# RRr89/Shared_SIMD_Scan

Measured on AMD Instinct MI355X. Metric: scanned values/sec + achieved HBM GB/s, 1e9 x 9-bit column (equality scan, bitmap + hit count out), higher is better.
Workload: dtype u32; 1 GPU; scan_eq ONE 1e+09x9bit column in 1 row-range shard(s) of <= 1000000000 rows, column=mod5, key=3; rows_total=1000000000, bits=9, parallelism=row-range shards x1

## Files before the change

shared_simd_scan_amd/csrc/kernels/in_list.hpp:

```cpp
#pragma once

#include "scan.hpp"

namespace mi355 {

template <int C, int AUX_, int VPL>
__global__ __launch_bounds__(kBlockThreads) void in_kernel(ScanArgs a)
{
    using G = ScanGeom<C, VPL>;
    constexpr int WORDS = G::WORDS;
    constexpr int AUX = AUX_ & 15;
    constexpr int NTS = store_policy_of(AUX_);
    constexpr bool BITSET = C <= 16;
    constexpr int SET_BYTES = BITSET ? ((1 << (C < 16 ? C : 16)) + 7) / 8 : 16;
    __shared__ __attribute__((aligned(16))) uint8_t lds[kWavesPerBlock][G::LDS_BYTES];
    __shared__ __attribute__((aligned(16))) uint32_t set_words[(SET_BYTES + 3) / 4];
    __shared__ __attribute__((aligned(16))) uint8_t mlds[kWavesPerBlock][1024];

    const int lane = threadIdx.x & 63;
    const int wave = __builtin_amdgcn_readfirstlane(threadIdx.x >> 6);
    uint8_t *lds_wave = lds[wave];
    const TileCtx<C, VPL> tc(a.n);
    const uint64_t stride = (uint64_t)gridDim.x * kWavesPerBlock;
    uint64_t tile = (uint64_t)blockIdx.x * kWavesPerBlock + wave;
// ... 19 lines not shown
    }
    const uint8_t *set_bytes = (const uint8_t *)set_words;

    uint32_t hits = 0;
    uint32_t res[WORDS];
    uint64_t prev = ~0ull;
    uint8_t *const out_lane = a.out + lane * (WORDS * 4);
    while (tile < tc.ntiles) {
        asm volatile("s_waitcnt vmcnt(0)" ::: "memory");
        uint32_t w[G::LANE_DWORDS];
        read_lane_data<C, VPL>(lds_wave, lane, w);
        uint32_t mcur[WORDS];
        if (a.and_mask && tile < tc.nfull) {
#pragma unroll
            for (int j = 0; j < WORDS; j++) mcur[j] = ((const uint32_t *)(mlds_wave + lane * (WORDS * 4)))[j];
        }
        asm volatile("s_waitcnt lgkmcnt(0)" ::: "memory");
        if (prev != ~0ull) store_words<WORDS, NTS>(out_lane + prev * G::BITMAP_BYTES, res);
        const uint64_t next = tile + stride;
        if (next < tc.ntiles) issue_tile(next);

        uint32_t xs[VPL];
        extract_all<C, VPL, 0, G::LANE_DWORDS>(w, xs);
        if constexpr (BITSET) {
#pragma unroll
            for (int j = 0; j < WORDS; j++) {
                uint32_t acc = 0;
#pragma unroll
                for (int k = 31; k >= 0; k--) {
                    const uint32_t x = xs[32 * j + k];
                    const uint32_t bit = (set_bytes[x >> 3] >> (x & 7)) & 1u;
                    acc = (acc << 1) | bit;
                }
                res[j] = acc;
            }
        } else {
            uint32_t m[WORDS];
#pragma unroll
            for (int j = 0; j < WORDS; j++) m[j] = 0;
            for (uint32_t k = 0; k < P; k++) {
                const uint32_t key = __builtin_amdgcn_readfirstlane((uint32_t)a.keys_dev[k]);
#pragma unroll
                for (int j = 0; j < WORDS; j++) {
                    uint32_t acc = 0;
#pragma unroll
                    for (int i = 31; i >= 0; i--) acc = (acc << 1) | (xs[32 * j + i] == key ? 1u : 0u);
                    m[j] |= acc;
                }
            }
#pragma unroll
            for (int j = 0; j < WORDS; j++) res[j] = m[j];
        }
        const uint32_t inv = a.invert;
#pragma unroll
        for (int j = 0; j < WORDS; j++) res[j] ^= inv;
        if (tile < tc.nfull) {
            if (a.and_mask) {
#pragma unroll
                for (int j = 0; j < WORDS; j++) res[j] &= mcur[j];
            }
#pragma unroll
            for (int j = 0; j < WORDS; j++) hits += __builtin_popcount(res[j]);
            prev = tile;
        } else {
            const int64_t left = (int64_t)(tc.n - tile * G::TILE_VALUES) - (int64_t)lane * VPL;
            const int nbytes = left <= 0 ? 0 : (int)((left >= VPL ? VPL : left) + 7) / 8;
            if (a.and_mask) {
                const uint8_t *mp = a.and_mask + tile * G::BITMAP_BYTES + lane * (WORDS * 4);
#pragma unroll
                for (int j = 0; j < WORDS; j++) {
                    uint32_t mm = 0;
#pragma unroll
                    for (int b = 0; b < 4; b++)
                        if (4 * j + b < nbytes) mm |= (uint32_t)mp[4 * j + b] << (8 * b);
                    res[j] &= mm;
                }
            }
            hits += tc.finish_tail(tile, res, out_lane + tile * G::BITMAP_BYTES, 1, lane);
            prev = ~0ull;
        }
        tile = next;
    }
    if (prev != ~0ull) store_words<WORDS, NTS>(out_lane + prev * G::BITMAP_BYTES, res);
    if (a.hits) hits_add(a, 0, wave_sum(hits), lane);
    hits_finalize(a, 1, lane);
}

}
```

shared_simd_scan_amd/csrc/kernels/scan.hpp:

```cpp
#pragma once

#include "tile.hpp"

namespace mi355 {

template <int C, int VPL> struct TileCtx {
    using G = ScanGeom<C, VPL>;
    uint64_t n, ntiles, nfull, data_bytes;
    uint32_t llc_inv, llc_lim;
    __device__ __forceinline__ TileCtx(uint64_t n_, uint32_t llc_inv_ = 0, uint32_t llc_lim_ = 0) : n(n_), llc_inv(llc_inv_), llc_lim(llc_lim_)
    {
        ntiles = (n + G::TILE_VALUES - 1) / G::TILE_VALUES;
        nfull = n / G::TILE_VALUES;
        data_bytes = (n * C + 7) / 8;
    }
    template <int AUX> __device__ __forceinline__ void issue(const uint8_t *packed, uint64_t t, uint8_t *lds_wave, int lane) const
    {
        if constexpr (AUX != 0) {
            if (llc_inv != 0 && (uint32_t)((t * G::TILE_BYTES) >> kLlcGranuleShift) * llc_inv <= llc_lim) {
                issue_as<0>(packed, t, lds_wave, lane);
                return;
            }
        }
        issue_as<AUX>(packed, t, lds_wave, lane);
    }
    template <int AUX> __device__ __forceinline__ void issue_as(const uint8_t *packed, uint64_t t, uint8_t *lds_wave, int lane) const
    {
        const uint8_t *src = packed + t * G::TILE_BYTES;
        if (t < nfull)
            dma_tile_full<G::TILE_BYTES, AUX>(src, lds_wave, lane);
        else
            dma_tile_partial<G::TILE_BYTES, AUX>(src, data_bytes - t * G::TILE_BYTES, lds_wave, lane);
    }
    template <bool HAVE_NBYTES = false>
    __device__ __forceinline__ void load_bitmap_words(const uint8_t *bits, uint64_t t, int lane, uint32_t (&m)[VPL / 32], uint64_t have_nbytes = 0) const
    {
        constexpr int WORDS = G::WORDS;
        const uint64_t at = t * G::BITMAP_BYTES + (uint64_t)lane * (WORDS * 4);
        if (t < nfull) {
#pragma unroll
            for (int j = 0; j < WORDS; j++) m[j] = ((const uint32_t *)(bits + at))[j];
        } else {
            const uint64_t nbytes = HAVE_NBYTES ? have_nbytes : (n + 7) / 8;
#pragma unroll
            for (int j = 0; j < WORDS; j++) {
                uint32_t v = 0;
#pragma unroll
                for (int b = 0; b < 4; b++)
                    if (at + 4 * j + b < nbytes) v |= (uint32_t)bits[at + 4 * j + b] << (8 * b);
                m[j] = v;
            }
        }
    }
    __device__ __forceinline__ uint32_t finish_tail(uint64_t t, uint32_t (&v)[VPL / 32], uint8_t *dst, uint64_t byte_stride, int lane,
                                                    bool store = true) const
    {
        const int64_t left = (int64_t)(n - t * G::TILE_VALUES) - (int64_t)lane * VPL;
        const int valid = left >= VPL ? VPL : (left <= 0 ? 0 : (int)left);
        const int nbytes = (valid + 7) / 8;
        uint32_t cnt = 0;
#pragma unroll
        for (int j = 0; j < VPL / 32; j++) {
            v[j] &= tail_mask(valid, j);
            cnt += __builtin_popcount(v[j]);
#pragma unroll
            for (int b = 0; b < 4; b++)
                if (store && 4 * j + b < nbytes) dst[(uint64_t)(4 * j + b) * byte_stride] = (uint8_t)(v[j] >> (8 * b));
        }
        return cnt;
    }
};

template <int C, int VPL, int K> constexpr int burst_occ()
{
    using G = ScanGeom<C, VPL>;
    constexpr int mask_bytes = (K * G::BITMAP_BYTES + 1023) / 1024 * 1024;
    constexpr int table = narrow_k<C>() ? (1 << (narrow_k<C>() * C)) : 16;
    constexpr int lds = kCuLdsBytes / (4 * (G::LDS_BYTES + mask_bytes) + table + 64);
    constexpr int cap = narrow_k<C>() ? 4 : 8;
    return lds > cap ? cap : (lds < 1 ? 1 : lds);
}

template <int C, int MODE, int AUX_, int VPL, int K>
__global__ __launch_bounds__(kBlockThreads, (burst_occ<C, VPL, K>())) void scan_burst_kernel(ScanArgs a)
{
    using G = ScanGeom<C, VPL>;
    static_assert(MODE == kModeEq || MODE == kModeRange, "MODE");
    constexpr int WORDS = G::WORDS;
    constexpr int AUX = AUX_ & 15;
    constexpr int NTS = store_policy_of(AUX_);
    __shared__ __attribute__((aligned(16))) uint8_t lds[kWavesPerBlock][G::LDS_BYTES];
    constexpr int LK = narrow_k<C>();
    __shared__ __attribute__((aligned(16))) uint8_t nlut[LK ? (1 << (LK * C)) : 16];
    constexpr int MASK_DMA = (K * G::BITMAP_BYTES + 1023) / 1024;
    __shared__ __attribute__((aligned(16))) uint8_t mlds[kWavesPerBlock][MASK_DMA * 1024];

    const int lane = threadIdx.x & 63;
    const int wave = __builtin_amdgcn_readfirstlane(threadIdx.x >> 6);
    uint8_t *lds_wave = lds[wave];
    uint8_t *mlds_wave = mlds[wave];
    const TileCtx<C, VPL> tc(a.n, a.llc_inv, a.llc_lim);
    const uint64_t nchunks = (tc.ntiles + K - 1) / K;
    const uint64_t stride = (uint64_t)gridDim.x * kWavesPerBlock;
    uint64_t chunk = (uint64_t)blockIdx.x * kWavesPerBlock + wave;

    uint32_t key[2] = {a.key[0], a.key[1]};
    uint32_t hits = 0;
    uint8_t *const out_lane = a.out + lane * (WORDS * 4);
    const bool store = a.out != nullptr;
    const uint8_t *const mask = a.and_mask;
    const uint32_t mop = a.mask_op, inv = a.invert;
    auto combine = [mop](uint32_t r, uint32_t m) -> uint32_t {
        return mop == 0 ? (r & m) : mop == 1 ? (r | m) : mop == 2 ? (r ^ m) : (m & ~r);
    };

    uint32_t res[K][WORDS];
    uint64_t pend_chunk = 0;
    int pend_n = 0;

    if (chunk < nchunks) tc.template issue<AUX>(a.packed, chunk * K, lds_wave, lane);
    if constexpr (LK > 0) {
        constexpr uint32_t fmask = (1u << C) - 1u;
        for (uint32_t e = threadIdx.x; e < (1u << (LK * C)); e += kBlockThreads) {
            uint32_t m = 0;
#pragma unroll
            for (int j = 0; j < LK; j++) {
                const uint32_t f = (e >> (j * C)) & fmask;
                const bool hit = (MODE == kModeRange) ? (f - key[0]) <= key[1] : f == key[0];
                m |= (hit ? 1u : 0u) << j;
            }
            nlut[e] = (uint8_t)m;
        }
        __syncthreads();
    }

    while (chunk < nchunks) {
        const uint64_t tfirst = chunk * K;
        int nfull_here = 0;
#pragma unroll
        for (int k = 0; k < K; k++) {
            const uint64_t tile = tfirst + k;
            if (tile < tc.ntiles) {
                asm volatile("s_waitcnt vmcnt(0)" ::: "memory");
                uint32_t w[G::LANE_DWORDS];
                read_lane_data<C, VPL>(lds_wave, lane, w);
                uint32_t mcur[WORDS];
                if (k > 0 && mask) {
#pragma unroll
                    for (int j = 0; j < WORDS; j++) mcur[j] = ((const uint32_t *)(mlds_wave + k * G::BITMAP_BYTES + lane * (WORDS * 4)))[j];
                }
                asm volatile("s_waitcnt lgkmcnt(0)" ::: "memory");
                if (k == 0) {
                    if (pend_n && store) {
                        uint8_t *dst = out_lane + pend_chunk * K * G::BITMAP_BYTES;
#pragma unroll
                        for (int q = 0; q < K; q++)
                            if (q < pend_n) store_words<WORDS, NTS>(dst + q * G::BITMAP_BYTES, res[q]);
                    }
                    pend_n = 0;
                    if (mask) {
                        const uint64_t mbytes = (tc.nfull > tfirst ? (tc.nfull - tfirst < K ? tc.nfull - tfirst : K) : 0) * G::BITMAP_BYTES;
                        const uint8_t *src = mask + tfirst * G::BITMAP_BYTES;
#pragma unroll
                        for (int q = 0; q < MASK_DMA; q++) {
                            const uint32_t o = q * 1024 + lane * 16;
                            if (o < mbytes) __builtin_amdgcn_global_load_lds(MI355_GPTR(src + o), MI355_LPTR(mlds_wave + q * 1024), 16, 0, 0);
                        }
                    }
                }
                const uint64_t next = (k + 1 < K && tile + 1 < tc.ntiles) ? tile + 1 : (chunk + stride) * K;
                const bool have_next = next < tc.ntiles && (k + 1 < K || chunk + stride < nchunks);
                if (have_next) tc.template issue<AUX>(a.packed, next, lds_wave, lane);
                uint32_t r1[1][WORDS];
                if constexpr (LK > 0) {
                    decode_words_narrow<C, VPL, LK, 0, G::LANE_DWORDS>(w, r1, nlut);
                } else {
                    const uint32_t key8[kMaxKeysPerPass] = {key[0], key[1], 0, 0, 0, 0, 0, 0};
                    decode_words<C, VPL, 0, 1, MODE, G::LANE_DWORDS>(w, r1, key8);
                }
#pragma unroll
                for (int j = 0; j < WORDS; j++) r1[0][j] ^= inv;
                if (tile < tc.nfull) {
                    if (mask) {
                        if (k == 0) {
                            if (have_next && next < tc.nfull)
                                asm volatile("s_waitcnt vmcnt(%0)" ::"n"(G::DMA_INSTRS) : "memory");
                            else
                                asm volatile("s_waitcnt vmcnt(0)" ::: "memory");
#pragma unroll
                            for (int j = 0; j < WORDS; j++) mcur[j] = ((const uint32_t *)(mlds_wave + lane * (WORDS * 4)))[j];
                            asm volatile("s_waitcnt lgkmcnt(0)" ::: "memory");
                        }
#pragma unroll
                        for (int j = 0; j < WORDS; j++) r1[0][j] = combine(r1[0][j], mcur[j]);
                    }
#pragma unroll
                    for (int j = 0; j < WORDS; j++) {
                        hits += __builtin_popcount(r1[0][j]);
                        res[k][j] = r1[0][j];
                    }
                    nfull_here = k + 1;
                } else {
                    if (mask) {
                        const uint8_t *mp = mask + tile * G::BITMAP_BYTES + lane * (WORDS * 4);
                        const int64_t left = (int64_t)(tc.n - tile * G::TILE_VALUES) - (int64_t)lane * VPL;
                        const int nbytes = left <= 0 ? 0 : (int)((left >= VPL ? VPL : left) + 7) / 8;
#pragma unroll
                        for (int j = 0; j < WORDS; j++) {
                            uint32_t m = 0;
#pragma unroll
                            for (int b = 0; b < 4; b++)
                                if (4 * j + b < nbytes) m |= (uint32_t)mp[4 * j + b] << (8 * b);
                            r1[0][j] = combine(r1[0][j], m);
                        }
                    }
                    hits += tc.finish_tail(tile, r1[0], out_lane + tile * G::BITMAP_BYTES, 1, lane, store);
                }
            }
        }
        pend_chunk = chunk;
        pend_n = nfull_here;
        chunk += stride;
    }
    if (pend_n && store) {
        uint8_t *dst = out_lane + pend_chunk * K * G::BITMAP_BYTES;
#pragma unroll
        for (int q = 0; q < K; q++)
            if (q < pend_n) store_words<WORDS, NTS>(dst + q * G::BITMAP_BYTES, res[q]);
    }
    if (a.hits) hits_add(a, 0, wave_sum(hits), lane);
    hits_finalize(a, 1, lane);
}

template <int C, int AUX_, int VPL>
__global__ __launch_bounds__(kBlockThreads, (burst_occ<C, VPL, 1>() > 1 ? burst_occ<C, VPL, 1>() / 2 : 1)) void scan2_kernel(ScanArgs a)
{
    using G = ScanGeom<C, VPL>;
    constexpr int WORDS = G::WORDS;
    constexpr int AUX = AUX_ & 15;
    constexpr int NTS = store_policy_of(AUX_);
    __shared__ __attribute__((aligned(16))) uint8_t lds[kWavesPerBlock][2][G::LDS_BYTES];

    const int lane = threadIdx.x & 63;
    const int wave = __builtin_amdgcn_readfirstlane(threadIdx.x >> 6);
    uint8_t *lds1 = lds[wave][0], *lds2 = lds[wave][1];
    const TileCtx<C, VPL> tc(a.n);
    const uint64_t stride = (uint64_t)gridDim.x * kWavesPerBlock;
    uint64_t tile = (uint64_t)blockIdx.x * kWavesPerBlock + wave;
    const uint32_t k1[kMaxKeysPerPass] = {a.key[0], a.key[1], 0, 0, 0, 0, 0, 0};
    const uint32_t k2[kMaxKeysPerPass] = {a.key2[0], a.key2[1], 0, 0, 0, 0, 0, 0};
    const uint32_t inv1 = a.invert, inv2 = a.invert2, mop = a.mask_op;
    auto combine = [mop](uint32_t p2, uint32_t p1) -> uint32_t {
        return mop == 0 ? (p2 & p1) : mop == 1 ? (p2 | p1) : mop == 2 ? (p2 ^ p1) : (p1 & ~p2);
    };
    uint32_t hits = 0;
    uint8_t *const out_lane = a.out + lane * (WORDS * 4);
    const bool store = a.out != nullptr;
    uint32_t res[WORDS];
    uint64_t prev = ~0ull;

    auto issue = [&](uint64_t t) {
        tc.template issue<AUX>(a.packed, t, lds1, lane);
        tc.template issue<AUX>(a.packed2, t, lds2, lane);
    };
    if (tile < tc.ntiles) issue(tile);
    while (tile < tc.ntiles) {
        asm volatile("s_waitcnt vmcnt(0)" ::: "memory");
        uint32_t w1[G::LANE_DWORDS], w2[G::LANE_DWORDS];
        read_lane_data<C, VPL>(lds1, lane, w1);
        read_lane_data<C, VPL>(lds2, lane, w2);
        asm volatile("s_waitcnt lgkmcnt(0)" ::: "memory");
        if (prev != ~0ull && store) store_words<WORDS, NTS>(out_lane + prev * G::BITMAP_BYTES, res);
        const uint64_t next = tile + stride;
        if (next < tc.ntiles) issue(next);
        uint32_t r1[1][WORDS], r2[1][WORDS];
        decode_words<C, VPL, 0, 1, kModeRange, G::LANE_DWORDS>(w1, r1, k1);
        decode_words<C, VPL, 0, 1, kModeRange, G::LANE_DWORDS>(w2, r2, k2);
#pragma unroll
        for (int j = 0; j < WORDS; j++) res[j] = combine(r2[0][j] ^ inv2, r1[0][j] ^ inv1);
        if (tile < tc.nfull) {
#pragma unroll
            for (int j = 0; j < WORDS; j++) hits += __builtin_popcount(res[j]);
            prev = tile;
        } else {
            hits += tc.finish_tail(tile, res, out_lane + tile * G::BITMAP_BYTES, 1, lane, store);
            prev = ~0ull;
        }
        tile = next;
    }
    if (prev != ~0ull && store) store_words<WORDS, NTS>(out_lane + prev * G::BITMAP_BYTES, res);
    if (a.hits) hits_add(a, 0, wave_sum(hits), lane);
    hits_finalize(a, 1, lane);
}

__device__ __forceinline__ void transpose4x4_bytes(const uint32_t (&r)[4], uint32_t (&c)[4])
{
    const uint32_t t0 = __builtin_amdgcn_perm(r[1], r[0], 0x05010400u);
    const uint32_t t1 = __builtin_amdgcn_perm(r[1], r[0], 0x07030602u);
    const uint32_t t2 = __builtin_amdgcn_perm(r[3], r[2], 0x05010400u);
    const uint32_t t3 = __builtin_amdgcn_perm(r[3], r[2], 0x07030602u);
    c[0] = __builtin_amdgcn_perm(t2, t0, 0x05040100u);
    c[1] = __builtin_amdgcn_perm(t2, t0, 0x07060302u);
    c[2] = __builtin_amdgcn_perm(t3, t1, 0x05040100u);
    c[3] = __builtin_amdgcn_perm(t3, t1, 0x07060302u);
}

}
```

shared_simd_scan_amd/csrc/kernels/tile.hpp:

```cpp
#pragma once

#include <hip/hip_runtime.h>
#include <stdint.h>

#include "../switches.hpp"

namespace mi355 {

typedef uint32_t u32x4 __attribute__((ext_vector_type(4)));
typedef uint32_t u32x2 __attribute__((ext_vector_type(2)));

#define MI355_GPTR(p) ((const __attribute__((address_space(1))) void *)(p))
#define MI355_LPTR(p) ((__attribute__((address_space(3))) void *)(p))

constexpr int kWavesPerBlock = 4;
constexpr int kBlockThreads = kWavesPerBlock * 64;
constexpr int kCuLdsBytes = 160 * 1024;
constexpr int kMaxKeysPerPass = 8;
constexpr uint64_t value_reach(unsigned c, uint64_t count) { return (c < 32 && count > (1ull << c)) ? (1ull << c) : count; }
constexpr int kMaxKeys = 1024;

template <int C, int VPL> struct ScanGeom {
    static_assert(VPL == 32 || VPL == 64 || VPL == 128, "VPL");
    static constexpr int WORDS = VPL / 32;
// ... 334 lines not shown
{
    Unaligned64 v;
    v.lo = lo;
    v.hi = hi;
    *(Unaligned64 *)dst = v;
}

constexpr int store_policy_of(int aux) { return (aux & 32) ? 2 : ((aux & 16) ? 1 : 0); }

template <int WORDS, int NT = 0> __device__ __forceinline__ void store_words(uint8_t *dst, const uint32_t (&v)[WORDS])
{
    if constexpr (WORDS == 4) {
        u32x4 t = {v[0], v[1], v[2], v[3]};
        if constexpr (NT == 2) {
            asm volatile("global_store_dwordx4 %0, %1, off sc1" ::"v"(dst), "v"(t) : "memory");
        } else if constexpr (NT == 1) __builtin_nontemporal_store(t, (u32x4 *)dst); else *(u32x4 *)dst = t;
    } else if constexpr (WORDS == 2) {
        u32x2 t = {v[0], v[1]};
        if constexpr (NT == 2) {
            asm volatile("global_store_dwordx2 %0, %1, off sc1" ::"v"(dst), "v"(t) : "memory");
        } else if constexpr (NT == 1) __builtin_nontemporal_store(t, (u32x2 *)dst); else *(u32x2 *)dst = t;
    } else {
        if constexpr (NT) __builtin_nontemporal_store(v[0], (uint32_t *)dst); else *(uint32_t *)dst = v[0];
    }
}

constexpr int kHitSlots = 64;
constexpr int kDoneGroups = 16;
constexpr int kScratchWords = kHitSlots * kMaxKeys + 8 + kDoneGroups * 16;
constexpr int kScratchDone = kHitSlots * kMaxKeys;
constexpr int kScratchGroupDone = kScratchDone + 8;

__device__ __forceinline__ void hits_add(const ScanArgs &a, uint32_t k, uint32_t wave_total, int lane)
{
    if (lane == 0 && wave_total)
        __hip_atomic_fetch_add(a.scratch + (blockIdx.x % kHitSlots) * kMaxKeys + k, (unsigned long long)wave_total,
                               __ATOMIC_RELAXED, __HIP_MEMORY_SCOPE_AGENT);
}

__device__ __forceinline__ void hits_finalize(const ScanArgs &a, uint32_t P, int lane)
{
    if (!a.hits) return;
    __shared__ uint32_t s_last;
    asm volatile("s_waitcnt vmcnt(0)" ::: "memory");
    __syncthreads();
    if (threadIdx.x == 0) {
        const uint32_t g = blockIdx.x % kDoneGroups;
        const uint32_t in_group = (gridDim.x - g + kDoneGroups - 1) / kDoneGroups;
        const uint32_t ngroups = gridDim.x < (unsigned)kDoneGroups ? gridDim.x : (unsigned)kDoneGroups;
        unsigned long long *const gdone = a.scratch + kScratchGroupDone + g * 16;
        uint32_t last = 0;
        if (__hip_atomic_fetch_add(gdone, 1ull, __ATOMIC_RELAXED, __HIP_MEMORY_SCOPE_AGENT) == (unsigned long long)in_group - 1) {
            __hip_atomic_store(gdone, 0ull, __ATOMIC_RELAXED, __HIP_MEMORY_SCOPE_AGENT);
            last = __hip_atomic_fetch_add(a.scratch + kScratchDone, 1ull, __ATOMIC_RELAXED, __HIP_MEMORY_SCOPE_AGENT) == (unsigned long long)ngroups - 1;
        }
        s_last = last;
    }
    __syncthreads();
    if (s_last) {
        const uint32_t nslots = gridDim.x < (unsigned)kHitSlots ? gridDim.x : (unsigned)kHitSlots;
        if (P <= 16u) {
            for (uint32_t k = threadIdx.x >> 6; k < P; k += kBlockThreads / 64) {
                const unsigned long long v = (uint32_t)lane < nslots
                                                 ? __hip_atomic_exchange(a.scratch + (uint32_t)lane * kMaxKeys + k, 0ull, __ATOMIC_RELAXED, __HIP_MEMORY_SCOPE_AGENT)
                                                 : 0ull;
                const unsigned long long lo = wave_sum((uint32_t)(v & 0xffffffull)), mid = wave_sum((uint32_t)((v >> 24) & 0xffffffull)),
                                         hi = wave_sum((uint32_t)(v >> 48));
                if (lane == 0) a.hits[k] = lo + (mid << 24) + (hi << 48);
            }
            if (threadIdx.x == 0) __hip_atomic_store(a.scratch + kScratchDone, 0ull, __ATOMIC_RELAXED, __HIP_MEMORY_SCOPE_AGENT);
            return;
        }
        for (uint32_t k = threadIdx.x; k < P; k += kBlockThreads) {
            unsigned long long v = 0;
#pragma unroll 8
            for (uint32_t sl = 0; sl < nslots; sl++)
                v += __hip_atomic_exchange(a.scratch + sl * kMaxKeys + k, 0ull, __ATOMIC_RELAXED, __HIP_MEMORY_SCOPE_AGENT);
            a.hits[k] = v;
        }
        if (threadIdx.x == 0) __hip_atomic_store(a.scratch + kScratchDone, 0ull, __ATOMIC_RELAXED, __HIP_MEMORY_SCOPE_AGENT);
    }
}

__device__ __forceinline__ void block_hits_clear(uint32_t *s_hits)
{
    for (uint32_t k = threadIdx.x; k < (uint32_t)kMaxKeys; k += kBlockThreads) s_hits[k] = 0;
}
__device__ __forceinline__ void block_hits_add8(uint32_t *s_hits, uint32_t kbase, uint32_t P, const uint32_t (&cnt)[8], int lane)
{
    uint32_t p0 = cnt[0] | (cnt[1] << 16), p1 = cnt[2] | (cnt[3] << 16), p2 = cnt[4] | (cnt[5] << 16), p3 = cnt[6] | (cnt[7] << 16);
    p0 = wave_sum(p0);
    p1 = wave_sum(p1);
    p2 = wave_sum(p2);
    p3 = wave_sum(p3);
    if (lane == 0) {
        const uint32_t v[8] = {p0 & 0xffff, p0 >> 16, p1 & 0xffff, p1 >> 16, p2 & 0xffff, p2 >> 16, p3 & 0xffff, p3 >> 16};
#pragma unroll
        for (int q = 0; q < 8; q++)
            if (kbase + q < P && v[q]) atomicAdd(&s_hits[kbase + q], v[q]);
    }
}

__device__ __forceinline__ void block_hits_flush(const ScanArgs &a, uint32_t *s_hits, uint32_t P)
{
    __syncthreads();
    for (uint32_t k = threadIdx.x; k < P; k += blockDim.x) {
        const uint32_t v = s_hits[k];
        if (v)
            __hip_atomic_fetch_add(a.scratch + (blockIdx.x % kHitSlots) * kMaxKeys + k, (unsigned long long)v, __ATOMIC_RELAXED,
                                   __HIP_MEMORY_SCOPE_AGENT);
    }
}

template <int C, int LK, int J, int GI, int NW>
__device__ __forceinline__ void narrow_step(const uint32_t (&w)[NW], uint32_t &acc, const uint8_t *table)
{
    constexpr int FIRST = LK * GI;
    constexpr int LEN = (32 - FIRST) < LK ? (32 - FIRST) : LK;
    uint32_t m = table[extract_at<(32 * J + FIRST) * C, LEN * C, NW>(w)];
    if constexpr (LEN < LK) m &= (1u << LEN) - 1u;
    acc = (acc << LEN) | m;
    if constexpr (GI > 0) narrow_step<C, LK, J, GI - 1, NW>(w, acc, table);
}

template <int C, int VPL, int LK, int J, int NW>
__device__ __forceinline__ void decode_words_narrow(const uint32_t (&w)[NW], uint32_t (&res)[1][VPL / 32], const uint8_t *table)
{
    uint32_t acc = 0;
    narrow_step<C, LK, J, (32 + LK - 1) / LK - 1, NW>(w, acc, table);
    res[0][J] = acc;
    if constexpr (J + 1 < VPL / 32) decode_words_narrow<C, VPL, LK, J + 1, NW>(w, res, table);
}

}
```

shared_simd_scan_amd/csrc/predicates/columns.hpp:

```cpp
#pragma once

#include "../kernels.hpp"
#include "../kernels/rt_column.hpp"

namespace mi355 {

struct ColumnsArgs {
    ScanArgs s;
    uint32_t c2;
    uint32_t nts;
    uint32_t lo, span;
    int64_t lo64;
    uint64_t span64;
};

constexpr int kColumnsMaskLds = 1024;

constexpr int columns_vpl(int C, bool same) { return same ? scan_vpl(C, kModeRange) : 32; }
template <int C1, int VPL, bool SAME> constexpr uint32_t columns_wave_lds(uint32_t c2)
{
    return (uint32_t)ScanGeom<C1, VPL>::LDS_BYTES + (SAME ? 1u : 2u) * ((64u * VPL * c2 / 8 + 1023u) / 1024u * 1024u) + (uint32_t)kColumnsMaskLds;
}
template <int C1, int VPL, bool SAME> constexpr uint32_t columns_block_lds(uint32_t c2)
{
// ... 88 lines not shown
    uint32_t res[WORDS];
    uint64_t prev = ~0ull;
    auto store_prev = [&]() {
        uint8_t *dst = out_lane + prev * G::BITMAP_BYTES;
        if (nts == 2)
            store_words<WORDS, 2>(dst, res);
        else if (nts == 1)
            store_words<WORDS, 1>(dst, res);
        else
            store_words<WORDS, 0>(dst, res);
    };

    auto issue = [&](uint64_t t, uint8_t *dst2) {
        tc.template issue<AUX>(s.packed, t, lds1, lane);
        if constexpr (SAME) {
            tc.template issue<AUX>(s.packed2, t, dst2, lane);
        } else {
            const uint64_t first = t * tile_bytes2;
            const uint8_t *src = s.packed2 + first;
            const uint64_t left = data_bytes2 - first;
            const uint32_t lim = left < tile_bytes2 ? (uint32_t)left : tile_bytes2;
#pragma unroll
            for (int j = 0; j < 8; j++) {
                const uint32_t o = j * 1024 + lane * 16;
                if ((uint32_t)j * 1024u < tile_bytes2 && o < lim) __builtin_amdgcn_global_load_lds(MI355_GPTR(src + o), MI355_LPTR(dst2 + j * 1024), 16, 0, AUX);
            }
        }
        if (mask && t < tc.nfull && (uint32_t)lane * 16u < MASK_TILE)
            __builtin_amdgcn_global_load_lds(MI355_GPTR(mask + t * MASK_TILE + lane * 16), MI355_LPTR(mlds), 16, 0, 0);
    };
    static_assert(SAME || VPL == 32, "run-time widths: the DMA loop above covers 8 KiB");

    if (tile < tc.ntiles) issue(tile, lds2);
    while (tile < tc.ntiles) {
        asm volatile("s_waitcnt vmcnt(0)" ::: "memory");
        uint32_t w1[G::LANE_DWORDS], w2[SAME ? G::LANE_DWORDS : 1], mw[WORDS] = {};
        read_lane_data<C1, VPL>(lds1, lane, w1);
        if constexpr (SAME) read_lane_data<C1, VPL>(lds2, lane, w2);
        const bool full = tile < tc.nfull;
        if (mask && full) {
#pragma unroll
            for (int j = 0; j < WORDS; j++) mw[j] = ((const uint32_t *)(mlds + lane * (WORDS * 4)))[j];
        }
        asm volatile("s_waitcnt lgkmcnt(0)" ::: "memory");
        if (prev != ~0ull && store) store_prev();
        const uint64_t next = tile + stride;
        if (next < tc.ntiles) issue(next, lds2_next);
        columns_words<C1, VPL, SAME, WIDE, 0, G::LANE_DWORDS>(w1, w2, lds2 + (uint32_t)lane * (VPL / 8u * c2), c2, vmask2, pred, res);
        if constexpr (!SAME) {
            uint8_t *const t2 = lds2;
            lds2 = lds2_next;
            lds2_next = t2;
        }
#pragma unroll
        for (int j = 0; j < WORDS; j++) res[j] ^= inv;
        if (full) {
            if (mask) {
#pragma unroll
                for (int j = 0; j < WORDS; j++) res[j] = combine(res[j], mw[j]);
            }
#pragma unroll
            for (int j = 0; j < WORDS; j++) hits += __builtin_popcount(res[j]);
            prev = tile;
        } else {
            if (mask) {
                const uint8_t *mp = mask + tile * MASK_TILE + lane * (WORDS * 4);
                const int64_t left = (int64_t)(tc.n - tile * G::TILE_VALUES) - (int64_t)lane * VPL;
                const int nbytes = left <= 0 ? 0 : (int)((left >= VPL ? VPL : left) + 7) / 8;
#pragma unroll
                for (int j = 0; j < WORDS; j++) {
                    uint32_t m = 0;
#pragma unroll
                    for (int b = 0; b < 4; b++)
                        if (4 * j + b < nbytes) m |= (uint32_t)mp[4 * j + b] << (8 * b);
                    res[j] = combine(res[j], m);
                }
            }
            hits += tc.finish_tail(tile, res, out_lane + tile * G::BITMAP_BYTES, 1, lane, store);
            prev = ~0ull;
        }
        tile = next;
    }
    if (prev != ~0ull && store) store_prev();
    if (s.hits) hits_add(s, 0, wave_sum(hits), lane);
    hits_finalize(s, 1, lane);
}

}
```

shared_simd_scan_amd/csrc/semijoin/semijoin.hpp:

```cpp
#pragma once

#include "../kernels.hpp"

namespace mi355 {

struct SemiArgs {
    ScanArgs s;
    const uint8_t *set;
    uint32_t set_bytes;
    uint32_t limit;
    uint32_t last_keep;
};

constexpr uint32_t kSemiMaskLds = 1024;
constexpr uint32_t kSemiLdsSlack = 64;
constexpr int kSemiGlobalMinBits = 20;

template <int C> constexpr uint32_t semijoin_static_lds()
{
    return (uint32_t)kWavesPerBlock * ((uint32_t)ScanGeom<C, scan_vpl(C, kModeEq)>::LDS_BYTES + kSemiMaskLds);
}
constexpr uint64_t semijoin_lds_max_bits()
{
    constexpr uint32_t widest = semijoin_static_lds<32>() > semijoin_static_lds<16>() ? semijoin_static_lds<32>() : semijoin_static_lds<16>();
// ... 70 lines not shown
        uint32_t w[G::LANE_DWORDS];
        read_lane_data<C, VPL>(lds_wave, lane, w);
        uint32_t mcur[WORDS];
        if (mask && tile < tc.nfull) {
#pragma unroll
            for (int j = 0; j < WORDS; j++) mcur[j] = ((const uint32_t *)(mlds_wave + lane * (WORDS * 4)))[j];
        }
        asm volatile("s_waitcnt lgkmcnt(0)" ::: "memory");
        if (prev != ~0ull && store) store_words<WORDS, NTS>(out_lane + prev * G::BITMAP_BYTES, res);
        const uint64_t next = tile + stride;
        if (next < tc.ntiles) {
            if (mask && next < tc.nfull && lane * 16 < G::BITMAP_BYTES)
                __builtin_amdgcn_global_load_lds(MI355_GPTR(mask + next * G::BITMAP_BYTES + lane * 16), MI355_LPTR(mlds_wave), 16, 0, 0);
            tc.template issue<AUX>(a.s.packed, next, lds_wave, lane);
        }

        uint32_t xs[VPL];
        extract_all<C, VPL, 0, G::LANE_DWORDS>(w, xs);
        if constexpr (LDS_SET) {
#pragma unroll
            for (int j = 0; j < WORDS; j++) {
                uint32_t acc = 0;
#pragma unroll
                for (int k = 31; k >= 0; k--) {
                    const uint32_t v = xs[32 * j + k];
                    const uint32_t at = (v >> 3) < zero_byte ? (v >> 3) : zero_byte;
                    const uint32_t bit = (set[at] >> (v & 7)) & 1u;
                    acc = (acc << 1) | bit;
                }
                res[j] = acc;
            }
        } else {
            uint32_t b[VPL];
#pragma unroll
            for (int k = 0; k < VPL; k++) {
                const uint32_t v = xs[k];
                const uint32_t x = v < limit ? v : limit;
                b[k] = set[x >> 3];
            }
            __builtin_amdgcn_sched_barrier(0);
#pragma unroll
            for (int j = 0; j < WORDS; j++) {
                uint32_t acc = 0;
#pragma unroll
                for (int k = 31; k >= 0; k--) {
                    const uint32_t v = xs[32 * j + k];
                    const uint32_t x = v < limit ? v : limit;
                    const uint32_t bit = (b[32 * j + k] >> (x & 7)) & (v <= limit ? 1u : 0u);
                    acc = (acc << 1) | bit;
                }
                res[j] = acc;
            }
        }
#pragma unroll
        for (int j = 0; j < WORDS; j++) res[j] ^= inv;
        if (tile < tc.nfull) {
            if (mask) {
#pragma unroll
                for (int j = 0; j < WORDS; j++) res[j] &= mcur[j];
            }
#pragma unroll
            for (int j = 0; j < WORDS; j++) hits += __builtin_popcount(res[j]);
            prev = tile;
        } else {
            if (mask) {
                const int64_t left = (int64_t)(tc.n - tile * G::TILE_VALUES) - (int64_t)lane * VPL;
                const int nbytes = left <= 0 ? 0 : (int)((left >= VPL ? VPL : left) + 7) / 8;
                const uint8_t *mp = mask + tile * G::BITMAP_BYTES + lane * (WORDS * 4);
#pragma unroll
                for (int j = 0; j < WORDS; j++) {
                    uint32_t mm = 0;
#pragma unroll
                    for (int q = 0; q < 4; q++)
                        if (4 * j + q < nbytes) mm |= (uint32_t)mp[4 * j + q] << (8 * q);
                    res[j] &= mm;
                }
            }
            hits += tc.finish_tail(tile, res, out_lane + tile * G::BITMAP_BYTES, 1, lane, store);
            prev = ~0ull;
        }
        tile = next;
    }
    if (prev != ~0ull && store) store_words<WORDS, NTS>(out_lane + prev * G::BITMAP_BYTES, res);
    if (a.s.hits) hits_add(a.s, 0, wave_sum(hits), lane);
    hits_finalize(a.s, 1, lane);
}

template <int C, int AUX_> __device__ __forceinline__ void semijoin_first_tile(const SemiArgs &a, uint8_t *lds_wave, uint8_t *mlds_wave)
{
    constexpr int VPL = scan_vpl(C, kModeEq);
    using G = ScanGeom<C, VPL>;
    const int lane = threadIdx.x & 63;
    const int wave = __builtin_amdgcn_readfirstlane(threadIdx.x >> 6);
    const TileCtx<C, VPL> tc(a.s.n);
    const uint64_t tile = (uint64_t)blockIdx.x * kWavesPerBlock + wave;
    if (tile >= tc.ntiles) return;
    if (a.s.and_mask && tile < tc.nfull && lane * 16 < G::BITMAP_BYTES)
        __builtin_amdgcn_global_load_lds(MI355_GPTR(a.s.and_mask + tile * G::BITMAP_BYTES + lane * 16), MI355_LPTR(mlds_wave), 16, 0, 0);
    tc.template issue<AUX_ & 15>(a.s.packed, tile, lds_wave, lane);
}

template <int C, int AUX_> __global__ __launch_bounds__(kBlockThreads) void semijoin_lds_kernel(SemiArgs a)
{
    using G = ScanGeom<C, scan_vpl(C, kModeEq)>;
    __shared__ __attribute__((aligned(16))) uint8_t lds[kWavesPerBlock][G::LDS_BYTES];
    __shared__ __attribute__((aligned(16))) uint8_t mlds[kWavesPerBlock][kSemiMaskLds];
    const int wave = __builtin_amdgcn_readfirstlane(threadIdx.x >> 6);
    semijoin_first_tile<C, AUX_>(a, lds[wave], mlds[wave]);
    const uint8_t *const set_lds = semijoin_stage_set(a);
    semijoin_tiles<C, AUX_, true>(a, set_lds, lds[wave], mlds[wave]);
}

template <int C, int AUX_> __global__ __launch_bounds__(kBlockThreads) void semijoin_global_kernel(SemiArgs a)
{
    static_assert(C >= kSemiGlobalMinBits, "narrower columns reach no set beyond the LDS tier");
    using G = ScanGeom<C, scan_vpl(C, kModeEq)>;
    __shared__ __attribute__((aligned(16))) uint8_t lds[kWavesPerBlock][G::LDS_BYTES];
    __shared__ __attribute__((aligned(16))) uint8_t mlds[kWavesPerBlock][kSemiMaskLds];
    const int wave = __builtin_amdgcn_readfirstlane(threadIdx.x >> 6);
    semijoin_first_tile<C, AUX_>(a, lds[wave], mlds[wave]);
    semijoin_tiles<C, AUX_, false>(a, a.set, lds[wave], mlds[wave]);
}

}
```

Before: 5109 billion values/s.

## Split burst scan into branch-free full rounds plus tail, fuse hit finalize

Restructures the burst scan loop so every wave first runs a fixed number of full K-tile rounds with no per-tile bounds or tail checks, then handles leftover tiles one at a time in a separate loop. Separately, it replaces the per-wave hits_add plus hits_finalize with a block-level reduction and a single packed atomic per block that counts arrivals and sums hits in one 64-bit word across group and top counters. The aim is to cut branch and bounds overhead in the hot loop and reduce atomic traffic and kernel-end synchronisation. The cost is extra code complexity, a __syncthreads at kernel end, and reliance on the packed count fitting within the stated static bounds.

```diff
diff --git a/shared_simd_scan_amd/csrc/kernels/in_list.hpp b/shared_simd_scan_amd/csrc/kernels/in_list.hpp
--- a/shared_simd_scan_amd/csrc/kernels/in_list.hpp
+++ b/shared_simd_scan_amd/csrc/kernels/in_list.hpp
@@ -125,8 +125,7 @@
         tile = next;
     }
     if (prev != ~0ull) store_words<WORDS, NTS>(out_lane + prev * G::BITMAP_BYTES, res);
-    if (a.hits) hits_add(a, 0, wave_sum(hits), lane);
-    hits_finalize(a, 1, lane);
+    hits_one(a, hits, lane);
 }
 
 }
diff --git a/shared_simd_scan_amd/csrc/kernels/scan.hpp b/shared_simd_scan_amd/csrc/kernels/scan.hpp
--- a/shared_simd_scan_amd/csrc/kernels/scan.hpp
+++ b/shared_simd_scan_amd/csrc/kernels/scan.hpp
@@ -1,6 +1,8 @@
 #pragma once
 
 #include "tile.hpp"
+
+#include "scan_split.hpp"
 
 namespace mi355 {
 
@@ -100,9 +102,12 @@
     uint8_t *lds_wave = lds[wave];
     uint8_t *mlds_wave = mlds[wave];
     const TileCtx<C, VPL> tc(a.n, a.llc_inv, a.llc_lim);
-    const uint64_t nchunks = (tc.ntiles + K - 1) / K;
-    const uint64_t stride = (uint64_t)gridDim.x * kWavesPerBlock;
-    uint64_t chunk = (uint64_t)blockIdx.x * kWavesPerBlock + wave;
+    const uint64_t W = (uint64_t)gridDim.x * kWavesPerBlock;
+    const uint64_t wid = (uint64_t)blockIdx.x * kWavesPerBlock + wave;
+    const uint64_t R = scan_full_rounds(tc.nfull, K, W);
+    const uint64_t tail0 = scan_tail_first(R, K, W);
+    uint64_t tail_step = 0;
+    uint64_t tail = scan_tail_tile(tail0, W, wid, 0);
 
     uint32_t key[2] = {a.key[0], a.key[1]};
     uint32_t hits = 0;
@@ -115,10 +120,21 @@
     };
 
     uint32_t res[K][WORDS];
-    uint64_t pend_chunk = 0;
+    uint8_t *pend_dst = nullptr;
     int pend_n = 0;
-
-    if (chunk < nchunks) tc.template issue<AUX>(a.packed, chunk * K, lds_wave, lane);
+    auto flush = [&]() {
+        if (pend_n && store) {
+#pragma unroll
+            for (int q = 0; q < K; q++)
+                if (q < pend_n) store_words<WORDS, NTS>(pend_dst + q * G::BITMAP_BYTES, res[q]);
+        }
+        pend_n = 0;
+    };
+
+    if (R > 0)
+        tc.template issue<AUX>(a.packed, scan_round_chunk(W, wid, 0) * K, lds_wave, lane);
+    else if (tail < tc.ntiles)
+        tc.template issue<AUX>(a.packed, tail, lds_wave, lane);
     if constexpr (LK > 0) {
         constexpr uint32_t fmask = (1u << C) - 1u;
         for (uint32_t e = threadIdx.x; e < (1u << (LK * C)); e += kBlockThreads) {
@@ -134,102 +150,134 @@
         __syncthreads();
     }
 
-    while (chunk < nchunks) {
-        const uint64_t tfirst = chunk * K;
-        int nfull_here = 0;
+    for (uint64_t r = 0; r < R; r++) {
+        const uint64_t tfirst = scan_round_chunk(W, wid, r) * K;
 #pragma unroll
         for (int k = 0; k < K; k++) {
             const uint64_t tile = tfirst + k;
-            if (tile < tc.ntiles) {
-                asm volatile("s_waitcnt vmcnt(0)" ::: "memory");
-                uint32_t w[G::LANE_DWORDS];
-                read_lane_data<C, VPL>(lds_wave, lane, w);
-                uint32_t mcur[WORDS];
-                if (k > 0 && mask) {
-#pragma unroll
-                    for (int j = 0; j < WORDS; j++) mcur[j] = ((const uint32_t *)(mlds_wave + k * G::BITMAP_BYTES + lane * (WORDS * 4)))[j];
-                }
-                asm volatile("s_waitcnt lgkmcnt(0)" ::: "memory");
-                if (k == 0) {
-                    if (pend_n && store) {
-                        uint8_t *dst = out_lane + pend_chunk * K * G::BITMAP_BYTES;
-#pragma unroll
-                        for (int q = 0; q < K; q++)
-                            if (q < pend_n) store_words<WORDS, NTS>(dst + q * G::BITMAP_BYTES, res[q]);
-                    }
-                    pend_n = 0;
-                    if (mask) {
-                        const uint64_t mbytes = (tc.nfull > tfirst ? (tc.nfull - tfirst < K ? tc.nfull - tfirst : K) : 0) * G::BITMAP_BYTES;
-                        const uint8_t *src = mask + tfirst * G::BITMAP_BYTES;
-#pragma unroll
-                        for (int q = 0; q < MASK_DMA; q++) {
-                            const uint32_t o = q * 1024 + lane * 16;
-                            if (o < mbytes) __builtin_amdgcn_global_load_lds(MI355_GPTR(src + o), MI355_LPTR(mlds_wave + q * 1024), 16, 0, 0);
-                        }
+            asm volatile("s_waitcnt vmcnt(0)" ::: "memory");
+            uint32_t w[G::LANE_DWORDS];
+            read_lane_data<C, VPL>(lds_wave, lane, w);
+            uint32_t mcur[WORDS];
+            if (k > 0 && mask) {
+#pragma unroll
+                for (int j = 0; j < WORDS; j++) mcur[j] = ((const uint32_t *)(mlds_wave + k * G::BITMAP_BYTES + lane * (WORDS * 4)))[j];
+            }
+            asm volatile("s_waitcnt lgkmcnt(0)" ::: "memory");
+            if (k == 0) {
+                flush();
+                if (mask) {
+                    const uint8_t *src = mask + tfirst * G::BITMAP_BYTES;
+#pragma unroll
+                    for (int q = 0; q < MASK_DMA; q++) {
+                        const uint32_t o = q * 1024 + lane * 16;
+                        if (o < (uint32_t)(K * G::BITMAP_BYTES)) __builtin_amdgcn_global_load_lds(MI355_GPTR(src + o), MI355_LPTR(mlds_wave + q * 1024), 16, 0, 0);
                     }
                 }
-                const uint64_t next = (k + 1 < K && tile + 1 < tc.ntiles) ? tile + 1 : (chunk + stride) * K;
-                const bool have_next = next < tc.ntiles && (k + 1 < K || chunk + stride < nchunks);
-                if (have_next) tc.template issue<AUX>(a.packed, next, lds_wave, lane);
-                uint32_t r1[1][WORDS];
-                if constexpr (LK > 0) {
-                    decode_words_narrow<C, VPL, LK, 0, G::LANE_DWORDS>(w, r1, nlut);
-                } else {
-                    const uint32_t key8[kMaxKeysPerPass] = {key[0], key[1], 0, 0, 0, 0, 0, 0};
-                    decode_words<C, VPL, 0, 1, MODE, G::LANE_DWORDS>(w, r1, key8);
+            }
+            const bool last = k + 1 == K;
+            const uint64_t next = !last ? tile + 1 : (r + 1 < R ? scan_round_chunk(W, wid, r + 1) * K : tail);
+            const bool have_next = !last || r + 1 < R || tail < tc.ntiles;
+            if (have_next) tc.template issue<AUX>(a.packed, next, lds_wave, lane);
+            uint32_t r1[1][WORDS];
+            if constexpr (LK > 0) {
+                decode_words_narrow<C, VPL, LK, 0, G::LANE_DWORDS>(w, r1, nlut);
+            } else {
+                const uint32_t key8[kMaxKeysPerPass] = {key[0], key[1], 0, 0, 0, 0, 0, 0};
+                decode_words<C, VPL, 0, 1, MODE, G::LANE_DWORDS>(w, r1, key8);
+            }
+#pragma unroll
+            for (int j = 0; j < WORDS; j++) r1[0][j] ^= inv;
+            if (mask) {
+                if (k == 0) {
+                    if (have_next && next < tc.nfull)
+                        asm volatile("s_waitcnt vmcnt(%0)" ::"n"(G::DMA_INSTRS) : "memory");
+                    else
+                        asm volatile("s_waitcnt vmcnt(0)" ::: "memory");
+#pragma unroll
+                    for (int j = 0; j < WORDS; j++) mcur[j] = ((const uint32_t *)(mlds_wave + lane * (WORDS * 4)))[j];
+                    asm volatile("s_waitcnt lgkmcnt(0)" ::: "memory");
                 }
 #pragma unroll
-                for (int j = 0; j < WORDS; j++) r1[0][j] ^= inv;
-                if (tile < tc.nfull) {
-                    if (mask) {
-                        if (k == 0) {
-                            if (have_next && next < tc.nfull)
-                                asm volatile("s_waitcnt vmcnt(%0)" ::"n"(G::DMA_INSTRS) : "memory");
-                            else
-                                asm volatile("s_waitcnt vmcnt(0)" ::: "memory");
-#pragma unroll
-                            for (int j = 0; j < WORDS; j++) mcur[j] = ((const uint32_t *)(mlds_wave + lane * (WORDS * 4)))[j];
-                            asm volatile("s_waitcnt lgkmcnt(0)" ::: "memory");
-                        }
-#pragma unroll
-                        for (int j = 0; j < WORDS; j++) r1[0][j] = combine(r1[0][j], mcur[j]);
-                    }
-#pragma unroll
-                    for (int j = 0; j < WORDS; j++) {
-                        hits += __builtin_popcount(r1[0][j]);
-                        res[k][j] = r1[0][j];
-                    }
-                    nfull_here = k + 1;
-                } else {
-                    if (mask) {
-                        const uint8_t *mp = mask + tile * G::BITMAP_BYTES + lane * (WORDS * 4);
-                        const int64_t left = (int64_t)(tc.n - tile * G::TILE_VALUES) - (int64_t)lane * VPL;
-                        const int nbytes = left <= 0 ? 0 : (int)((left >= VPL ? VPL : left) + 7) / 8;
-#pragma unroll
-                        for (int j = 0; j < WORDS; j++) {
-                            uint32_t m = 0;
-#pragma unroll
-                            for (int b = 0; b < 4; b++)
-                                if (4 * j + b < nbytes) m |= (uint32_t)mp[4 * j + b] << (8 * b);
-                            r1[0][j] = combine(r1[0][j], m);
-                        }
-                    }
-                    hits += tc.finish_tail(tile, r1[0], out_lane + tile * G::BITMAP_BYTES, 1, lane, store);
+                for (int j = 0; j < WORDS; j++) r1[0][j] = combine(r1[0][j], mcur[j]);
+            }
+#pragma unroll
+            for (int j = 0; j < WORDS; j++) {
+                hits += __builtin_popcount(r1[0][j]);
+                res[k][j] = r1[0][j];
+            }
+        }
+        pend_dst = out_lane + tfirst * G::BITMAP_BYTES;
+        pend_n = K;
+    }
+
+    while (tail < tc.ntiles) {
+        const uint64_t tile = tail;
+        const bool whole = tile < tc.nfull;
+        asm volatile("s_waitcnt vmcnt(0)" ::: "memory");
+        uint32_t w[G::LANE_DWORDS];
+        read_lane_data<C, VPL>(lds_wave, lane, w);
+        asm volatile("s_waitcnt lgkmcnt(0)" ::: "memory");
+        flush();
+        if (mask && whole) {
+            const uint8_t *src = mask + tile * G::BITMAP_BYTES;
+#pragma unroll
+            for (int q = 0; q < (G::BITMAP_BYTES + 1023) / 1024; q++) {
+                const uint32_t o = q * 1024 + lane * 16;
+                if (o < (uint32_t)G::BITMAP_BYTES) __builtin_amdgcn_global_load_lds(MI355_GPTR(src + o), MI355_LPTR(mlds_wave + q * 1024), 16, 0, 0);
+            }
+        }
+        tail = scan_tail_tile(tail0, W, wid, ++tail_step);
+        const bool have_next = tail < tc.ntiles;
+        if (have_next) tc.template issue<AUX>(a.packed, tail, lds_wave, lane);
+        uint32_t r1[1][WORDS];
+        if constexpr (LK > 0) {
+            decode_words_narrow<C, VPL, LK, 0, G::LANE_DWORDS>(w, r1, nlut);
+        } else {
+            const uint32_t key8[kMaxKeysPerPass] = {key[0], key[1], 0, 0, 0, 0, 0, 0};
+            decode_words<C, VPL, 0, 1, MODE, G::LANE_DWORDS>(w, r1, key8);
+        }
+#pragma unroll
+        for (int j = 0; j < WORDS; j++) r1[0][j] ^= inv;
+        if (whole) {
+            if (mask) {
+                if (have_next && tail < tc.nfull)
+                    asm volatile("s_waitcnt vmcnt(%0)" ::"n"(G::DMA_INSTRS) : "memory");
+                else
+                    asm volatile("s_waitcnt vmcnt(0)" ::: "memory");
+                uint32_t mcur[WORDS];
+#pragma unroll
+                for (int j = 0; j < WORDS; j++) mcur[j] = ((const uint32_t *)(mlds_wave + lane * (WORDS * 4)))[j];
+                asm volatile("s_waitcnt lgkmcnt(0)" ::: "memory");
+#pragma unroll
+                for (int j = 0; j < WORDS; j++) r1[0][j] = combine(r1[0][j], mcur[j]);
+            }
+#pragma unroll
+            for (int j = 0; j < WORDS; j++) {
+                hits += __builtin_popcount(r1[0][j]);
+                res[0][j] = r1[0][j];
+            }
+            pend_dst = out_lane + tile * G::BITMAP_BYTES;
+            pend_n = 1;
+        } else {
+            if (mask) {
+                const uint8_t *mp = mask + tile * G::BITMAP_BYTES + lane * (WORDS * 4);
+                const int64_t left = (int64_t)(tc.n - tile * G::TILE_VALUES) - (int64_t)lane * VPL;
+                const int nbytes = left <= 0 ? 0 : (int)((left >= VPL ? VPL : left) + 7) / 8;
+#pragma unroll
+                for (int j = 0; j < WORDS; j++) {
+                    uint32_t m = 0;
+#pragma unroll
+                    for (int b = 0; b < 4; b++)
+                        if (4 * j + b < nbytes) m |= (uint32_t)mp[4 * j + b] << (8 * b);
+                    r1[0][j] = combine(r1[0][j], m);
                 }
             }
-        }
-        pend_chunk = chunk;
-        pend_n = nfull_here;
-        chunk += stride;
-    }
-    if (pend_n && store) {
-        uint8_t *dst = out_lane + pend_chunk * K * G::BITMAP_BYTES;
-#pragma unroll
-        for (int q = 0; q < K; q++)
-            if (q < pend_n) store_words<WORDS, NTS>(dst + q * G::BITMAP_BYTES, res[q]);
-    }
-    if (a.hits) hits_add(a, 0, wave_sum(hits), lane);
-    hits_finalize(a, 1, lane);
+            hits += tc.finish_tail(tile, r1[0], out_lane + tile * G::BITMAP_BYTES, 1, lane, store);
+        }
+    }
+    flush();
+    hits_one(a, hits, lane);
 }
 
 template <int C, int AUX_, int VPL>
@@ -289,8 +337,7 @@
         tile = next;
     }
     if (prev != ~0ull && store) store_words<WORDS, NTS>(out_lane + prev * G::BITMAP_BYTES, res);
-    if (a.hits) hits_add(a, 0, wave_sum(hits), lane);
-    hits_finalize(a, 1, lane);
+    hits_one(a, hits, lane);
 }
 
 __device__ __forceinline__ void transpose4x4_bytes(const uint32_t (&r)[4], uint32_t (&c)[4])
diff --git a/shared_simd_scan_amd/csrc/kernels/scan_split.hpp b/shared_simd_scan_amd/csrc/kernels/scan_split.hpp
--- /dev/null
+++ b/shared_simd_scan_amd/csrc/kernels/scan_split.hpp
@@ -0,0 +1,18 @@
+#pragma once
+
+#include <stdint.h>
+
+#if defined(__HIPCC__)
+#define MI355_SPLIT_FN __host__ __device__ constexpr
+#else
+#define MI355_SPLIT_FN constexpr
+#endif
+
+namespace mi355 {
+
+MI355_SPLIT_FN uint64_t scan_full_rounds(uint64_t nfull, uint32_t K, uint64_t W) { return K <= 1 ? 0 : nfull / K / W; }
+MI355_SPLIT_FN uint64_t scan_round_chunk(uint64_t W, uint64_t w, uint64_t r) { return r * W + w; }
+MI355_SPLIT_FN uint64_t scan_tail_first(uint64_t R, uint32_t K, uint64_t W) { return R * W * K; }
+MI355_SPLIT_FN uint64_t scan_tail_tile(uint64_t tail_first, uint64_t W, uint64_t w, uint64_t s) { return tail_first + s * W + w; }
+
+}
diff --git a/shared_simd_scan_amd/csrc/kernels/tile.hpp b/shared_simd_scan_amd/csrc/kernels/tile.hpp
--- a/shared_simd_scan_amd/csrc/kernels/tile.hpp
+++ b/shared_simd_scan_amd/csrc/kernels/tile.hpp
@@ -440,6 +440,40 @@
     }
 }
 
+constexpr int kHitsOneShift = 44;
+static_assert((1ull << kHitsOneShift) > 8ull * 288ull * 1000000000ull, "a launch's hits fit below the arrivals");
+static_assert((1ull << (64 - kHitsOneShift)) > 8ull * 256ull, "the arrivals of a 2048-block grid fit above the count");
+
+__device__ __forceinline__ void hits_one(const ScanArgs &a, uint32_t lane_hits, int lane)
+{
+    if (!a.hits) return;
+    __shared__ uint32_t s_wave_hits[kWavesPerBlock];
+    const uint32_t wave_total = wave_sum(lane_hits);
+    if (lane == 0) s_wave_hits[threadIdx.x >> 6] = wave_total;
+    __syncthreads();
+    if (threadIdx.x == 0) {
+        constexpr unsigned long long one = 1ull << kHitsOneShift, count_mask = one - 1;
+        unsigned long long total = 0;
+#pragma unroll
+        for (int w = 0; w < kWavesPerBlock; w++) total += s_wave_hits[w];
+        const uint32_t g = blockIdx.x % kDoneGroups;
+        const uint32_t in_group = (gridDim.x - g + kDoneGroups - 1) / kDoneGroups;
+        const uint32_t ngroups = gridDim.x < (unsigned)kDoneGroups ? gridDim.x : (unsigned)kDoneGroups;
+        unsigned long long *const gword = a.scratch + kScratchGroupDone + g * 16;
+        unsigned long long *const top = a.scratch + kScratchDone;
+        unsigned long long was = __hip_atomic_fetch_add(gword, one | total, __ATOMIC_RELAXED, __HIP_MEMORY_SCOPE_AGENT);
+        if ((was >> kHitsOneShift) == (unsigned long long)in_group - 1) {
+            __hip_atomic_store(gword, 0ull, __ATOMIC_RELAXED, __HIP_MEMORY_SCOPE_AGENT);
+            total += was & count_mask;
+            was = __hip_atomic_fetch_add(top, one | total, __ATOMIC_RELAXED, __HIP_MEMORY_SCOPE_AGENT);
+            if ((was >> kHitsOneShift) == (unsigned long long)ngroups - 1) {
+                __hip_atomic_store(top, 0ull, __ATOMIC_RELAXED, __HIP_MEMORY_SCOPE_AGENT);
+                a.hits[0] = total + (was & count_mask);
+            }
+        }
+    }
+}
+
 __device__ __forceinline__ void block_hits_clear(uint32_t *s_hits)
 {
     for (uint32_t k = threadIdx.x; k < (uint32_t)kMaxKeys; k += kBlockThreads) s_hits[k] = 0;
diff --git a/shared_simd_scan_amd/csrc/predicates/columns.hpp b/shared_simd_scan_amd/csrc/predicates/columns.hpp
--- a/shared_simd_scan_amd/csrc/predicates/columns.hpp
+++ b/shared_simd_scan_amd/csrc/predicates/columns.hpp
@@ -194,8 +194,7 @@
         tile = next;
     }
     if (prev != ~0ull && store) store_prev();
-    if (s.hits) hits_add(s, 0, wave_sum(hits), lane);
-    hits_finalize(s, 1, lane);
-}
-
-}
+    hits_one(s, hits, lane);
+}
+
+}
diff --git a/shared_simd_scan_amd/csrc/semijoin/semijoin.hpp b/shared_simd_scan_amd/csrc/semijoin/semijoin.hpp
--- a/shared_simd_scan_amd/csrc/semijoin/semijoin.hpp
+++ b/shared_simd_scan_amd/csrc/semijoin/semijoin.hpp
@@ -176,8 +176,7 @@
         tile = next;
     }
     if (prev != ~0ull && store) store_words<WORDS, NTS>(out_lane + prev * G::BITMAP_BYTES, res);
-    if (a.s.hits) hits_add(a.s, 0, wave_sum(hits), lane);
-    hits_finalize(a.s, 1, lane);
+    hits_one(a.s, hits, lane);
 }
 
 template <int C, int AUX_> __device__ __forceinline__ void semijoin_first_tile(const SemiArgs &a, uint8_t *lds_wave, uint8_t *mlds_wave)
```

Result: no change. 5151 billion values/s, median of 6 (+0.8%).
